# riveSunder/therldaisyworld

Hardware: AMD Instinct MI355X
Metric: cell-updates/sec (grid x batch), fused stencil+growth step (higher is better)
Workload: dtype f32

## Files before the change

### therldaisyworld_amd/csrc/dw_api.hip

```cpp
#include <hip/hip_runtime.h>

#include <cmath>
#include <cstdarg>
#include <cstdio>
#include <cstdlib>
#include <cstring>
#include <memory>
#include <new>
#include <type_traits>
#include <vector>

#include "../../include/daisyworld_hip.h"
#include "dw_kernels.hpp"
#include "dw_host_util.hpp"
#include "dw_plan.hpp"
#include "dw_series.hpp"

using namespace dw;

static thread_local char g_err[512] = "";

static int fail(int code, const char* fmt, ...) {
    va_list ap;
    va_start(ap, fmt);
// ... 439 lines not shown
        });
    } else {
        const int prec = p.precision == DW_PRECISION_F64 ? 2 : (ex ? 0 : 1);
        with_int<2, 0, 1>(prec, [&](auto PR) { generic(iL, iD, PR); });
    }
    HIPCHK(hipGetLastError());
    step_done(h, 0.0, true, true, constants);
    return DW_OK;
}

static int launch_forward_fused2_pw(dw_handle* h, const PairPw* row, StatsDev* trace) {
    const StepPlan& pl = h->plan;
    const StepOut o = step_out(h);
    const FusedGeom& g = pl.fgeom;
    const dim3 grid((unsigned)g.chunk * 8u);
    const plane_t *inL = h->L16[h->cur].get(), *inD = h->D16[h->cur].get();
    with_int<kFusedRot, kFusedOvl>(pl.fused_mode, [&](auto MODE) {
        hipLaunchKernelGGL((trace_pair_fast_pw<MODE>), grid, dim3(256), 0, h->stream, inL, inD, o.L, o.D, g, row, o.zero_me,
                           o.zero_n, trace);
    });
    HIPCHK(hipGetLastError());
    step_done(h, 0.0, false, true, true);
    return DW_OK;
}

static int temp_chunks(const dw_handle* h) {
    return (int)(((long long)h->prm.height * h->prm.width + kTempChunk - 1) / kTempChunk);
}
static size_t temp_part_bytes(const dw_handle* h) { return sizeof(TempPartial) * (size_t)h->prm.batch * temp_chunks(h); }

static int launch_temp_moments(dw_handle* h, bool current, double L, const PhysF64* row64, TempStatsDev* out) {
    const dw_params& p = h->prm;
    const int chunks = temp_chunks(h);
    const PhysF64 P = row64 ? PhysF64{} : make_f64(p, L);
    TempPartial* part = h->temp_part.get();
    auto reduce = [&](auto* iL, auto* iD) {
        with_bool(row64 != nullptr, [&](auto TABLE) {
            hipLaunchKernelGGL((temp_moments_pw<elem_t<decltype(iL)>, TABLE>), dim3((unsigned)chunks, (unsigned)p.batch), dim3(256),
                               0, h->stream, iL, iD, p.height, p.width, P, row64, part);
        });
    };
    if (current) with_planes(h, h->unq == OWN_CUR, h->cur, reduce);
    else with_derived_from(h, [&](auto* iL, auto* iD, auto) { reduce(iL, iD); });
    HIPCHK(hipGetLastError());
    hipLaunchKernelGGL(temp_moments_finish_pw, dim3((unsigned)((p.batch + 63) / 64)), dim3(64), 0, h->stream, part, p.batch, chunks,
                       (double)p.height * (double)p.width, out);
    HIPCHK(hipGetLastError());
    return DW_OK;
}

template <class F>
static auto with_fused_layout(const StepPlan& pl, F&& f) {
    if (pl.packed) return f(int_c<kFusedRot>{}, std::true_type{});
    return with_int<kFusedRot, kFusedRing, kFusedOvl>(pl.fused_mode, [&](auto MODE) { return f(MODE, std::false_type{}); });
}

static int launch_forward_fused2(dw_handle* h, double L1, double L2, unsigned int* pstats = nullptr,
                                 float thr_hi = 0.f, StatsDev* trace = nullptr) {
    const dw_params& p = h->prm;
    const StepPlan& pl = h->plan;
    const bool exact = p.precision == DW_PRECISION_EXACT;
    PhysF32 P1, P2;
    if (exact) derive_f32_pair(p, L1, L2, &P1, &P2);
    else { P1 = derive_f32(p, L1); P2 = derive_f32(p, L2); }
    const StepOut o = step_out(h);
    const FusedGeom& g = pl.fgeom;
    const dim3 grid((unsigned)g.chunk * 8u);
    const plane_t *inL = h->L16[h->cur].get(), *inD = h->D16[h->cur].get();
    auto exact_args = [&] {
        return FusedExactArgs{inL, inD, o.L, o.D, g, P1, lum_part(P2), o.zero_me, o.zero_n, pstats, thr_hi, make_f64(p, L1), L1, L2};
    };
    if (trace && exact) {
        const TraceExactArgs A{exact_args(), trace, h->sw.force_rescan ? 1 : 0};
        with_int<kFusedRot, kFusedOvl>(pl.fused_mode, [&](auto MODE) {
            with_bool(pl.sym_albedo, [&](auto SYM) {
                hipLaunchKernelGGL((trace_pair_exact<MODE, SYM>), grid, dim3(256), 0, h->stream, A);
            });
        });
    } else if (trace) {
        with_int<kFusedRot, kFusedOvl>(pl.fused_mode, [&](auto MODE) {
            hipLaunchKernelGGL((trace_pair_fast<MODE>), grid, dim3(256), 0, h->stream, inL, inD, o.L, o.D, g, P1, P2, o.zero_me,
                               o.zero_n, trace);
        });
    } else if (pl.fmt_planes && !pstats && !exact) {
        hipLaunchKernelGGL((step_stream_fused2_fmt_pw<kFusedOvl>), grid, dim3(256), 0, h->stream, inL, inD, o.L, o.D, g, P1, P2,
                           o.zero_me, o.zero_n);
    } else if (exact) {
        const FusedExactArgs A = exact_args();
        with_bool(pstats != nullptr, [&](auto STATS) {
            with_fused_layout(pl, [&](auto MODE, auto PACK) {
                with_bool(pl.sym_albedo, [&](auto SYM) {
                    hipLaunchKernelGGL((step_stream_fused2_exact<MODE, PACK, STATS, SYM>), grid, dim3(256), 0, h->stream, A);
                });
            });
        });
    } else {
        with_bool(pstats != nullptr, [&](auto STATS) {
            with_fused_layout(pl, [&](auto MODE, auto PACK) {
                hipLaunchKernelGGL((step_stream_fused2<MODE, PACK, STATS>), grid, dim3(256), 0, h->stream, inL, inD, o.L, o.D, g,
                                   P1, P2, o.zero_me, o.zero_n, pstats, thr_hi);
            });
        });
    }
    HIPCHK(hipGetLastError());
    step_done(h, L2, false);
    return DW_OK;
}

static int launch_agents(dw_handle* h, const int* d_action, int act_b, int act_n, bool standalone = false,
                         double* d_reward = nullptr, unsigned char* d_done = nullptr, unsigned char* d_ok = nullptr) {
    const dw_params& p = h->prm;
    if (p.n_agents == 0) return DW_OK;
    NEED(h->have_state, DW_ESTATE, "no state uploaded");
    NEED(h->have_agents, DW_ESTATE, "no agents uploaded (call dw_upload_agents or dw_init_random)");
    NEED(p.collision_mode == 0 || standalone, DW_EINVAL,
         "collision_mode=1: call dw_update_agents, apply the collision pass (it consumes the caller's RNG) to the "
         "downloaded agent states, upload them, then dw_step without actions");
    const int blocks = (p.batch + 63) / 64;
    with_planes(h, h->unq == OWN_CUR, h->cur, [&](auto* L, auto* D) {
        using T = elem_t<decltype(L)>;
        hipLaunchKernelGGL(agents_update<T>, dim3(blocks), dim3(64), 0, h->stream, L, D, h->idx.get(), h->st.get(), d_action,
                           act_b, act_n, p.batch, p.n_agents, p.height, p.width, p.agent_gamma,
                           p.collision_mode == 0 ? 1 : 0, d_reward, d_done, d_ok);
    });
    HIPCHK(hipGetLastError());
    return DW_OK;
}

static int stage_host_actions(dw_handle* h, const int32_t* action, int b, int n) {
    const dw_params& p = h->prm;
    NEED(b >= 0 && n >= 0 && b <= p.batch && n <= p.n_agents, DW_EINVAL,
         "action block %dx%d exceeds (B,N)=(%d,%d)", b, n, p.batch, p.n_agents);
    if ((size_t)b * n)
        HIPCHK(hipMemcpyAsync(h->action_tmp.get(), action, sizeof(int) * (size_t)b * n, hipMemcpyHostToDevice,
                              h->stream));
    return DW_OK;
}

static int clear_stats(dw_handle* h) {
    for (int i = 0; i < 2; ++i) HIPCHK(hipMemsetAsync(h->stats2[i].get(), 0, h->stats_bytes, h->stream));
    return DW_OK;
}

static void state_arrived(dw_handle* h, UnqOwner unq, UnqKind kind = UNQ_F64) {
    if (unq == OWN_CUR) h->unq_kind = kind;
    h->unq = unq;
    h->have_state = true;
    h->stepped = false;
    for (auto& sn : h->snap) sn.valid = false;
}

template <class T>
static auto init_random_into(dw_handle* h, uint64_t seed, T* L, T* D) {
    const dw_params& p = h->prm;
    if (int crc = clear_stats(h)) return crc;
    const int ncell = p.height * p.width;
    const dim3 g((unsigned)((ncell + kInitChunk - 1) / kInitChunk), (unsigned)p.batch);
    hipLaunchKernelGGL((init_random_cells<T>), g, dim3(256), 0, h->stream, L, D, ncell,
                       (long long)p.world_offset, (unsigned long long)seed, (float)p.light_proportion,
                       (float)p.dark_proportion, (float)p.initial_al, (float)p.initial_ad, h->stats2[h->sp].get());
    HIPCHK(hipGetLastError());
    if (p.n_agents) {
        const int bn = p.batch * p.n_agents;
        hipLaunchKernelGGL(init_random_agents, dim3((bn + 255) / 256), dim3(256), 0, h->stream, h->idx.get(), h->st.get(),
                           p.batch, p.n_agents, p.height, p.width, (long long)p.world_offset,
                           (unsigned long long)seed);
// ... 1613 lines not shown
        job(h->idx.get(), sn.idx.get(), sizeof(int) * 2 * bn);
        job(h->st.get(), sn.st.get(), sizeof(double) * bn);
    }
    if (sn.stepped && sn.unq != OWN_PREV) {
        job(h->L16[1 - h->cur].get(), sn.PL.get(), pb);
        job(h->D16[1 - h->cur].get(), sn.PD.get(), pb);
    }
    if (int rc = launch_copy_regions(h, J)) return rc;
    HIPCHK(hipMemsetAsync(h->stats2[1 - h->sp].get(), 0, h->stats_bytes, h->stream));
    h->unq = sn.unq;
    h->stepped = sn.stepped;
    h->L_last = sn.L_last;
    h->L_per_world = sn.L_per_world;
    h->P_per_world = sn.P_per_world;
    return DW_OK;
}

int dw_snapshot_save(dw_handle* h) { return dw_snapshot_save_slot(h, 0); }
int dw_snapshot_restore(dw_handle* h) { return dw_snapshot_restore_slot(h, 0); }


int dw_set_stream(dw_handle* h, void* hip_stream) {
    NEED(h, DW_EINVAL, "null handle");
    HIPCHK(hipSetDevice(h->prm.device));
    HIPCHK(hipStreamSynchronize(h->stream));
    if (h->own_stream) HIPCHK(hipStreamDestroy(h->stream));
    h->stream = reinterpret_cast<hipStream_t>(hip_stream);
    h->own_stream = false;
    return DW_OK;
}

int dw_sync(dw_handle* h) {
    NEED(h, DW_EINVAL, "null handle");
    HIPCHK(hipSetDevice(h->prm.device));
    HIPCHK(hipStreamSynchronize(h->stream));
    return DW_OK;
}

int dw_timer_start(dw_handle* h) {
    NEED(h, DW_EINVAL, "null handle");
    HIPCHK(hipSetDevice(h->prm.device));
    HIPCHK(hipEventRecord(h->ev0, h->stream));
    return DW_OK;
}

int dw_timer_stop(dw_handle* h, float* elapsed_ms) {
    NEED(h && elapsed_ms, DW_EINVAL, "null argument");
    HIPCHK(hipSetDevice(h->prm.device));
    HIPCHK(hipEventRecord(h->ev1, h->stream));
    HIPCHK(hipEventSynchronize(h->ev1));
    HIPCHK(hipEventElapsedTime(elapsed_ms, h->ev0, h->ev1));
    return DW_OK;
}

int dw_device_planes(dw_handle* h, int which, void** light, void** dark) {
    NEED(h && light && dark, DW_EINVAL, "null argument");
    NEED(which == DW_STATE_CURRENT || which == DW_STATE_PREVIOUS, DW_EINVAL, "bad state selector");
    const int buf = which == DW_STATE_CURRENT ? h->cur : 1 - h->cur;
    NEED(which != DW_STATE_CURRENT || cur_quantised(h), DW_ESTATE,
         "the current state is an un-quantised upload: it has no binary16 planes before the first step");
    *light = h->L16[buf].get();
    *dark = h->D16[buf].get();
    return DW_OK;
}

int dw_kernel_info(dw_handle* h, char* buf, size_t buflen) {
    NEED(h && buf && buflen, DW_EINVAL, "null argument");
    const dw_params& p = h->prm;
    const StepPlan& pl = h->plan;
    const char* prec = p.precision == DW_PRECISION_EXACT ? "exact" : (p.precision == DW_PRECISION_FAST ? "fast" : "f64");
    static const char* const halo_name[] = {"rotate", "dpp-old", "general", "packed"};
    if (pl.kind == STEP_STREAM) {
        const StripGeom& g = pl.sgeom;
        snprintf(buf, buflen,
                 "step_stream_%s<halo=%s> wave-strip=%dx256 cells, register window + DPP neighbours, %d-row blocks in "
                 "flight%s, %d strips, grid=%d x 256 threads (4 strips each), XCD-chunked",
                 prec, halo_name[pl.halo], g.SR,
                 p.precision == DW_PRECISION_EXACT ? DW_STREAM_RB_EXACT : DW_STREAM_RB_FAST,
                 p.precision == DW_PRECISION_EXACT ? ", in-wave float64 fix-up from an LDS queue" : "", g.nstrips,
                 g.chunk * 8);
        if (pl.allow_fuse) {
            const size_t n = std::strlen(buf);
            snprintf(buf + n, buflen - n, "; dw_step_n fuses step pairs (step_stream_fused2%s%s)",
                     p.precision == DW_PRECISION_EXACT ? "_exact" : "", pl.fmt_planes ? "_fmt_pw, format buffer accesses" : "");
        }
    } else if (pl.kind == STEP_TILED) {
        const int TR = (256 / pl.tcq) * pl.rpt;
        snprintf(buf, buflen,
                 "step_tiled<TCQ=%d,RPT=%d,%s> tile=%dx%d cells, %zu B LDS/workgroup, %d tiles, grid=%d x 256 threads, "
                 "XCD-chunked",
                 pl.tcq, pl.rpt, prec, TR, pl.tcq * 4, pl.tile_lds, pl.geom.ntiles, pl.geom.chunk * 8);
    } else {
        snprintf(buf, buflen, "step_generic<%s> one thread per cell, grid=(%d,%d) x 256 threads", prec,
                 (p.height * p.width + 255) / 256, p.batch);
    }
    {
        const size_t n = std::strlen(buf);
        snprintf(buf + n, buflen - n, pl.trace_pairs ? "; trace: step pairs" : "; trace: single steps");
    }
    {
        const size_t n = std::strlen(buf);
        snprintf(buf + n, buflen - n, pl.pw_stream ? "; per-world L: wave strips" : "; per-world L: generic");
    }
    {
        static const char* const form_name[] = {"launches per step", "workgroup (LDS)", "one wave per world"};
        const size_t n = std::strlen(buf);
        snprintf(buf + n, buflen - n, "; episode: %s; mlp episode: %s", form_name[episode_form(h)], form_name[episode_mlp_form(h)]);
    }
    {
        const size_t n = std::strlen(buf);
        snprintf(buf + n, buflen - n, "; ensemble episode: %s", ensemble_episode_wave(h) ? "one wave per world" : "launches per step");
    }
    {
        const size_t n = std::strlen(buf);
        snprintf(buf + n, buflen - n, "; episode trace: %s", episode_trace_wave(h) ? "one wave per world" : "launches per step");
    }
    if (pl.first_stream) {
        const size_t n = std::strlen(buf);
        snprintf(buf + n, buflen - n, "; first step: wave-strip=%dx256", pl.first_geom.SR);
    }
    if (h->sw.text[0]) {
        const size_t n = std::strlen(buf);
        snprintf(buf + n, buflen - n, "; switches[%s]", h->sw.text);
    }
    {
        const size_t n = std::strlen(buf);
        snprintf(buf + n, buflen - n, "; per-world constants: %s",
                 ensemble_pairs(h) ? "step pairs" : (pl.pw_stream ? "wave strips" : "generic"));
    }
    return DW_OK;
}

int dw_audit_tie_bound(dw_handle* h, double L, double out[4]) {
    NEED(h && out, DW_EINVAL, "null argument");
    const dw_params& p = h->prm;
    HIPCHK(hipSetDevice(p.device));
    NEED(h->have_state && cur_quantised(h), DW_ESTATE, "the audit needs a quantised current state");
    const StepPlan& pl = h->plan;
    int rc = ensure_scratch(h, 4 * sizeof(unsigned long long));
    if (rc) return rc;
    unsigned long long* d = reinterpret_cast<unsigned long long*>(h->scratch.get());
    HIPCHK(hipMemsetAsync(d, 0, 4 * sizeof(unsigned long long), h->stream));
    const dim3 g((unsigned)((p.height * p.width + 255) / 256), (unsigned)p.batch);
    hipLaunchKernelGGL(tie_audit, g, dim3(256), 0, h->stream, h->L16[h->cur].get(), h->D16[h->cur].get(), p.height, p.width,
                       derive_f32(p, L), make_f64(p, L), d, pl.sym_albedo && pl.kind == STEP_STREAM ? 1 : 0);
    HIPCHK(hipGetLastError());
    unsigned long long r[4];
    HIPCHK(hipMemcpyAsync(r, d, sizeof(r), hipMemcpyDeviceToHost, h->stream));
    HIPCHK(hipStreamSynchronize(h->stream));
    std::memcpy(&out[0], &r[0], sizeof(double));
    std::memcpy(&out[1], &r[1], sizeof(double));
    out[2] = (double)r[2];
    out[3] = (double)r[3];
    return DW_OK;
}

int dw_last_fixup_count(dw_handle* h, uint64_t* count) {
    NEED(h && count, DW_EINVAL, "null argument");
    HIPCHK(hipSetDevice(h->prm.device));
    std::vector<StatsDev> st((size_t)h->prm.batch + 1);
    HIPCHK(hipMemcpyAsync(st.data(), h->stats2[h->sp].get(), sizeof(StatsDev) * st.size(), hipMemcpyDeviceToHost, h->stream));
    HIPCHK(hipStreamSynchronize(h->stream));
    unsigned long long v = st[h->prm.batch].sum_l;
    for (int b = 0; b < h->prm.batch; ++b) v += st[b].reserved;
    *count = v;
    return DW_OK;
}
// ... 3 lines not shown
```

### therldaisyworld_amd/csrc/dw_kernels.hpp

```cpp
#pragma once
#include "dw_common.hpp"
#include "dw_step_generic.hpp"
#include "dw_step_tiled.hpp"
#include "dw_step_stream.hpp"
#include "dw_step_fused.hpp"
#include "dw_step_first.hpp"
#include "dw_step_per_world.hpp"
#include "dw_step_fused_pw.hpp"
#include "dw_episode.hpp"
#include "dw_episode_wave.hpp"
#include "dw_agents.hpp"
#include "dw_state_io.hpp"
#include "dw_agents_fused.hpp"
#include "dw_temp_moments.hpp"
#include "dw_episode_wave_pw.hpp"
#include "dw_episode_wave_stats_pw.hpp"
```

### therldaisyworld_amd/csrc/dw_plan.hpp

```cpp
#pragma once
#include <climits>
#include <cmath>
#include <cstddef>
#include <cstdio>
#include <cstdlib>
#include <cstring>

#include "../../include/daisyworld_hip.h"
#include "dw_types.hpp"

namespace dw {

struct Switches {
    bool no_sym = false, no_pack = false, no_fuse = false, no_ring = false, no_fmt_planes = false, no_episode_kernel = false,
         no_episode_wave = false, no_agent_fuse = false, no_agent_preapply = false, first_f64 = false,
         first_generic = false, force_rescan = false, test_hooks = false;
    int pack_min_strips = -1, strip_rows = 0, tile_rpt = 0, queue_cap = -1, mismatch_cap = -1, trace_rows = 0;
    double first_slack = -1.0;
    char kernel[16] = {0};
    char text[256] = {0};
};
inline const char* test_hook(const char* name) {
    return std::getenv("DW_TEST_HOOKS") ? std::getenv(name) : nullptr;
}
inline Switches read_switches() {
    Switches w;
    auto note = [&](const char* name, const char* val) {
        const size_t n = std::strlen(w.text);
        snprintf(w.text + n, sizeof(w.text) - n, "%s%s%s%s", n ? " " : "", name, val ? "=" : "", val ? val : "");
    };
    auto flag = [&](const char* name, bool& dst) { if (std::getenv(name)) { dst = true; note(name, nullptr); } };
    auto num = [&](const char* name, int& dst, bool test) {
        if (const char* e = test ? test_hook(name) : std::getenv(name)) { dst = std::atoi(e); note(name, e); }
    };
    w.test_hooks = std::getenv("DW_TEST_HOOKS") != nullptr;
    flag("DW_NO_SYM", w.no_sym); flag("DW_NO_PACK", w.no_pack); flag("DW_NO_FUSE", w.no_fuse); flag("DW_NO_RING", w.no_ring);
    flag("DW_NO_FMT_PLANES", w.no_fmt_planes);
    flag("DW_NO_EPISODE_KERNEL", w.no_episode_kernel); flag("DW_NO_EPISODE_WAVE", w.no_episode_wave);
    flag("DW_NO_AGENT_FUSE", w.no_agent_fuse); flag("DW_NO_AGENT_PREAPPLY", w.no_agent_preapply);
    flag("DW_FIRST_STEP_F64", w.first_f64); flag("DW_FIRST_GENERIC", w.first_generic);
    num("DW_PACK_MIN_STRIPS", w.pack_min_strips, false); num("DW_STRIP_ROWS", w.strip_rows, false);
    num("DW_TILE_RPT", w.tile_rpt, false);
    num("DW_TEST_QUEUE_CAP", w.queue_cap, true); num("DW_TEST_MISMATCH_CAP", w.mismatch_cap, true);
    num("DW_TEST_TRACE_ROWS", w.trace_rows, true);
    if (test_hook("DW_TEST_FORCE_RESCAN")) { w.force_rescan = true; note("DW_TEST_FORCE_RESCAN", nullptr); }
    if (const char* e = test_hook("DW_TEST_FIRST_SLACK")) { w.first_slack = std::atof(e); note("DW_TEST_FIRST_SLACK", e); }
    if (const char* e = std::getenv("DW_KERNEL")) { snprintf(w.kernel, sizeof(w.kernel), "%s", e); note("DW_KERNEL", e); }
    return w;
}

inline dw_params with_world_params(dw_params p, const dw_world_params& w) {
    p.p = w.p; p.g = w.g; p.S = w.S; p.sigma = w.sigma; p.gamma = w.gamma; p.q = w.q; p.q2 = w.q2; p.dt = w.dt;
    p.albedo_bare = w.albedo_bare; p.albedo_light = w.albedo_light; p.albedo_dark = w.albedo_dark;
    p.temp_optimal = w.temp_optimal;
    return p;
}
inline dw_world_params world_params_of(const dw_params& p) {
    return dw_world_params{p.p, p.g, p.S, p.sigma, p.gamma, p.q, p.q2, p.dt, p.albedo_bare, p.albedo_light, p.albedo_dark,
                           p.temp_optimal};
}
inline bool albedo_symmetric(double bare, double light, double dark) { return (dark - bare) == -(light - bare); }
inline bool worlds_symmetric(const dw_world_params* worlds, size_t B) {
    for (size_t b = 0; b < B; ++b)
        if (!albedo_symmetric(worlds[b].albedo_bare, worlds[b].albedo_light, worlds[b].albedo_dark)) return false;
    return true;
}

inline PhysF64 make_f64(const dw_params& p, double L) {
    PhysF64 P;
    P.p = p.p; P.g = p.g; P.S = p.S; P.sigma = p.sigma; P.gamma = p.gamma; P.q = p.q; P.q2 = p.q2;
    P.dt = p.dt; P.ab = p.albedo_bare; P.al = p.albedo_light; P.ad = p.albedo_dark;
    P.To = p.temp_optimal; P.L = L;
    const double e1 = std::exp(-1.0), e2 = std::exp(-2.0);
    const double s = 1.0 + 4.0 * e1 + 4.0 * e2;
    P.w0 = 1.0 / s; P.w1 = e1 / s; P.w2 = e2 / s;
    return P;
}

inline double cbeta_host(const dw_params& p) {
    const double cbeta = p.g * p.temp_optimal * p.temp_optimal;
    return cbeta > 1e-30 ? 1.0 / std::sqrt(cbeta) : 0x1p60;
}

inline void split_hi_lo(double v, double scale, float* hi, float* lo) {
    const double h = std::nearbyint(v * scale) / scale;
    *hi = (float)h;
    *lo = (float)(v - h);
}

inline float round_up(double v) {
    const float f = (float)v;
    return (double)f < v ? std::nextafterf(f, INFINITY) : f;
}

struct EConst { double c0l, c0d; };
inline EConst e_const(const dw_params& p, double L) {
    const double To4 = std::pow(p.temp_optimal, 4), K = p.S * L / p.sigma;
    const double e0 = K * (1.0 - p.albedo_bare * p.p) / To4 - 1.0;
    return EConst{e0 + p.q2 * (p.albedo_bare * p.p - p.albedo_light) / To4,
                  e0 + p.q2 * (p.albedo_bare * p.p - p.albedo_dark) / To4};
}

struct TieChain {
    double emin, emax, vlo;
    bool admissible;
    double ew;
    double kbmax;
    double pu, safety;
};
inline TieChain tie_chain(const dw_params& p, const EConst& c, double a1, double a2, double a3, double a4, double de) {
    const double u = std::ldexp(1.0, -24), kmax = 1000.0;
    TieChain t;
    const double pos = (std::fmax(a1, 0.0) + std::fmax(a2, 0.0)) * 8 * kmax + (std::fmax(a3, 0.0) + std::fmax(a4, 0.0)) * kmax;
    const double neg = (std::fmin(a1, 0.0) + std::fmin(a2, 0.0)) * 8 * kmax + (std::fmin(a3, 0.0) + std::fmin(a4, 0.0)) * kmax;
    t.emax = std::fmax(c.c0l, c.c0d) + pos;
    t.emin = std::fmin(c.c0l, c.c0d) + neg;
    const double vmin = 1.0 + t.emin, vmax = 1.0 + t.emax;
    t.admissible = vmin > 0.02;
    t.vlo = std::fmax(vmin, 0.02);
    const double smax = std::sqrt(std::fmax(vmax, t.vlo));
// ... 39 lines not shown
    P.a1 = (float)((double)P.a1h + P.a1l); P.a2 = (float)((double)P.a2h + P.a2l);
    P.a3 = (float)((double)P.a3h + P.a3l); P.a4 = (float)((double)P.a4h + P.a4l);
    P.c0ls = (float)((double)P.c0lh + P.c0ll); P.c0ds = (float)((double)P.c0dh + c0dl);
    const double kbe = cbeta_host(p);
    P.kbeta = (float)kbe;
    const PhysF64 P64 = make_f64(p, L);
    P.dw0 = (float)(p.dt * P64.w0); P.dw1 = (float)(p.dt * P64.w1); P.dw2 = (float)(p.dt * P64.w2);
    P.p = (float)p.p; P.ck = p.dt != 0.0 ? (float)(0.001 / p.dt) : 0.f;
    P.ngamma = (float)(-p.gamma);
    const double u = std::ldexp(1.0, -24);
    const double lo_mag = std::ldexp(1.0, -(hb + 1)) * 18.0 * kmax + std::ldexp(1.0, -(hb + 1));
    const double de_abs = 6.0 * u * lo_mag + 1e-9;
    const TieChain t = tie_chain(p, c0, a1, a2, a3, a4, de_abs);
    auto e_over_D2 = [&](double e) {
        const double v = std::fmax(1.0 + e, t.vlo), sv = std::sqrt(v), yv = std::sqrt(sv);
        const double D = kbe * (yv + 1.0) * (sv + 1.0);
        return std::fabs(e) / (D * D);
    };
    const double Ae = 2.0 * de_abs * std::fmax(e_over_D2(t.emin), e_over_D2(t.emax));
    double A0 = t.safety * (kmax * std::fabs(p.dt) * t.kbmax * Ae + 2e-6);
    if (!t.admissible) A0 = 1.0;
    const double eA = t.safety * 13.0 * u;
    const double eK0d = t.safety * (6.0 * std::fabs(p.p) + t.pu + t.kbmax + 8.0 * std::fabs(p.gamma)) * u;
    const double eK1d = t.safety * ((6.0 * std::fabs(p.p) + t.pu) * u + t.kbmax * (u + 2.0 * t.ew));
    P.tie_lo = (float)(0.5 - A0);
    if ((double)P.tie_lo > 0.5 - A0) P.tie_lo = std::nextafterf(P.tie_lo, -INFINITY);
    P.eA = round_up(eA);
    const float eK0 = round_up(eK0d), eK1 = round_up(eK1d);
    P.eK0s = p.dt < 0.0 ? eK0 : -eK0;
    P.eK1s = p.dt < 0.0 ? eK1 : -eK1;
    P.neK1s = -P.eK1s;
    P.eK01s = (float)((double)P.eK0s + (double)P.eK1s);
    if (std::fabs((double)P.eK01s) < std::fabs((double)P.eK0s + (double)P.eK1s))
        P.eK01s = std::nextafterf(P.eK01s, P.eK01s < 0.f ? -1.f : 1.f);
    return P;
}

inline void derive_f32_pair(const dw_params& p, double L1, double L2, PhysF32* P1, PhysF32* P2) {
    const PhysF32 a = derive_f32(p, L1), b = derive_f32(p, L2);
    const int hb = a.hi_bits < b.hi_bits ? a.hi_bits : b.hi_bits;
    *P1 = derive_f32(p, L1, hb);
    *P2 = derive_f32(p, L2, hb);
    const float tie_lo = P1->tie_lo < P2->tie_lo ? P1->tie_lo : P2->tie_lo;
    P1->tie_lo = tie_lo;
    P2->tie_lo = tie_lo;
}

inline FirstStepBound derive_first_bound(const dw_params& p, double L, const PhysF32& P, bool from_f64,
                                         double test_slack = -1.0) {
    const double u = std::ldexp(1.0, -24), iota = from_f64 ? u : 0.0;
    const double kmax = 1000.0;
    const double a1 = std::fabs((double)P.a1), a2 = std::fabs((double)P.a2), a3 = std::fabs((double)P.a3), a4 = std::fabs((double)P.a4);
    const EConst c0 = e_const(p, L);
    const double c0m = std::fmax(std::fabs(c0.c0l), std::fabs(c0.c0d));
    const double Mmax = (a1 + a2) * 8 * kmax + (a3 + a4) * kmax;
    const double de_max = (8.0 * u + iota) * Mmax + u * c0m;
    const TieChain t = tie_chain(p, c0, P.a1, P.a2, P.a3, P.a4, de_max);
    const double kbe = cbeta_host(p);
    const double Dmin = kbe * (std::sqrt(std::sqrt(t.vlo)) + 1.0) * (std::sqrt(t.vlo) + 1.0);
    const double kK = 5.0 * u + iota;
    const double safety = t.safety, pu = t.pu, kbmax = t.kbmax;
    FirstStepBound B;
    B.a1 = round_up(a1); B.a2 = round_up(a2); B.a3 = round_up(a3); B.a4 = round_up(a4);
    B.c_de = round_up(safety * (8.0 * u + iota) * (1.0 + 8.0 * u));
    B.c_c0 = round_up(safety * u * c0m);
    B.eK0 = round_up(safety * (pu + (kK + 2.0 * u) * std::fabs(p.p) + kbmax * u + ((kK + 3.0 * u) + u) * std::fabs(p.gamma)));
    B.eK1 = round_up(safety * (pu + (kK + 2.0 * u) * std::fabs(p.p) + kbmax * (u + 2.0 * t.ew)));
    B.cW = round_up(safety * 2.0 * kbmax / Dmin);
    B.eA = round_up(safety * ((kK + 3.0 * u) + u + (kK + u)));
    B.cS = round_up(safety * u);
    B.slack = t.admissible ? 4e-6f : 1.0f;
    if (test_slack > (double)B.slack) B.slack = (float)test_slack;
    return B;
}

enum StepKind { STEP_GENERIC, STEP_TILED, STEP_STREAM };
struct StepPlan {
    StepKind kind = STEP_GENERIC;
    int halo = 0;
    bool packed = false;
    bool allow_fuse = false;
    int fused_mode = kFusedOvl;
    bool fmt_planes = false;
    bool trace_pairs = false;
    bool sym_albedo = false;
    int tcq = 0, rpt = 0;
    Geom geom{};
    size_t tile_lds = 0;
    StripGeom sgeom{};
    FusedGeom fgeom{};
    int first_prec = 2;
    bool first_stream = false;
    FirstGeom first_geom{};
    bool need_fixq = false;
    bool pw_stream = false;
};

inline int halo_form(int W) { return W < 256 ? 3 : (W == 256 ? 0 : (W % 256 == 0 ? 1 : 2)); }

inline int strip_rows(long groups, int H, long target) {
    int sr = 64;
    while (sr > 8 && groups * ((H + sr - 1) / sr) < target) sr >>= 1;
    return H < sr ? H : sr;
}

inline int strip_rows_or_override(const Switches& sw, int cap, long groups, int H, long target) {
    if (sw.strip_rows < 1) return strip_rows(groups, H, target);
    const int want = sw.strip_rows < cap ? sw.strip_rows : cap;
    return H < want ? H : want;
}

inline StepPlan plan_steps(const dw_params& p, const Switches& sw) {
    StepPlan s;
    s.sym_albedo = albedo_symmetric(p.albedo_bare, p.albedo_light, p.albedo_dark) && !sw.no_sym;
    s.halo = halo_form(p.width);
    const int lpw = p.width / 4, wpr = lpw ? 64 / lpw : 0;
    const bool pack_shape = p.width >= 8 && p.width < 256 && wpr >= 1 && wpr * lpw * 10 >= 64 * 7 && !sw.no_pack;
    const long pack_strips = pack_shape ? (long)((p.batch + wpr - 1) / wpr) * ((p.height + 63) / 64) : 0;
    const bool packable = pack_shape && pack_strips >= (sw.pack_min_strips >= 0 ? sw.pack_min_strips : 512);
    const bool quads = p.precision != DW_PRECISION_F64 && p.width % 4 == 0;
    if (quads && (p.width >= 256 || packable) && std::strcmp(sw.kernel, "tiled") != 0) {
        s.kind = STEP_STREAM;
        s.packed = p.width < 256;
        StripGeom& g = s.sgeom;
        g.B = p.batch; g.H = p.height; g.W = p.width;
        g.ncs = (p.width + 255) / 256;
        g.lpw = s.packed ? lpw : 64;
        g.wpr = s.packed ? wpr : 1;
        const long groups = s.packed ? (p.batch + wpr - 1) / wpr : p.batch;
        g.SR = strip_rows_or_override(sw, INT_MAX, groups * g.ncs, p.height, 2048);
        g.nrs = (p.height + g.SR - 1) / g.SR;
        g.nstrips = (int)(groups * g.nrs * g.ncs);
        g.nwg = (g.nstrips + 3) / 4;
        g.chunk = (g.nwg + 7) / 8;
        g.qcap = kWaveQueueCap;
        int mcap = kMismatchCap;
        if (sw.queue_cap >= 0 && sw.queue_cap < kWaveQueueCap) g.qcap = sw.queue_cap;
        if (sw.mismatch_cap >= 0 && sw.mismatch_cap < kMismatchCap) mcap = sw.mismatch_cap;
        g.force_rescan = sw.force_rescan ? 1 : 0;
        s.allow_fuse = !sw.no_fuse;
        const bool ring = p.width == 1024 && !sw.no_ring;
        s.fused_mode = p.width <= 256 ? kFusedRot : (ring ? kFusedRing : kFusedOvl);
        FusedGeom& f = s.fgeom;
        f.B = p.batch; f.H = p.height; f.W = p.width;
        f.SR = g.SR;
        f.nrs = g.nrs;
        f.lpw = g.lpw; f.wpr = g.wpr;
        f.cols_per_strip = p.width <= 256 ? 256 : (ring ? 1024 : 248);
        f.ncs = s.packed ? 1 : (p.width + f.cols_per_strip - 1) / f.cols_per_strip;
        f.nstrips = (int)(groups * f.nrs * f.ncs);
        f.nwg = ring ? f.nstrips : (f.nstrips + 3) / 4;
        f.chunk = (f.nwg + 7) / 8;
        f.qcap = g.qcap;
        f.mcap = mcap;
        f.sure_need = 9 * p.n_agents + 9 * mcap + 1;
        s.trace_pairs = s.allow_fuse && !s.packed && s.fused_mode != kFusedRing;
        s.fmt_planes = p.precision == DW_PRECISION_FAST && s.allow_fuse && !s.packed && s.fused_mode == kFusedOvl && !sw.no_fmt_planes &&
                       (size_t)p.height * p.width * sizeof(plane_t) < ((size_t)1 << 31);
    } else if (quads && p.width >= 64) {
        s.kind = STEP_TILED;
        const int Wq = p.width / 4;
        if (Wq >= 64) {
            s.tcq = 64; s.rpt = 4;
            if (sw.tile_rpt == 2 || sw.tile_rpt == 4 || sw.tile_rpt == 8) s.rpt = sw.tile_rpt;
        }
        else if (Wq >= 32) { s.tcq = 32; s.rpt = 4; }
        else { s.tcq = 16; s.rpt = 2; }
        const int TR = (256 / s.tcq) * s.rpt;
        Geom& g = s.geom;
        g.B = p.batch; g.H = p.height; g.W = p.width; g.Wq = Wq;
        g.tiles_r = (p.height + TR - 1) / TR;
        g.tiles_c = (Wq + s.tcq - 1) / s.tcq;
        g.ntiles = p.batch * g.tiles_r * g.tiles_c;
        g.chunk = (g.ntiles + 7) / 8;
        g.qcap = kMaxFix;
        if (sw.queue_cap >= 0 && sw.queue_cap < kMaxFix) g.qcap = sw.queue_cap;
        s.tile_lds = (size_t)2 * (TR + 2) * (s.tcq + 2) * 4 * sizeof(float);
    }
    s.need_fixq = p.precision == DW_PRECISION_EXACT && s.kind == STEP_TILED;
    s.pw_stream = s.kind == STEP_STREAM && !s.packed;
    s.first_prec = p.precision == DW_PRECISION_FAST ? 1 : (p.precision == DW_PRECISION_EXACT && !sw.first_f64 ? 3 : 2);
    s.first_stream = (p.width % 256 == 0 || s.kind == STEP_STREAM) && s.first_prec != 2 && !sw.first_generic;
    if (s.first_stream) {
        FirstGeom& fg = s.first_geom;
        fg.B = p.batch; fg.H = p.height; fg.W = p.width;
        fg.lpw = s.packed ? lpw : 64;
        fg.wpr = s.packed ? wpr : 1;
        fg.ncs = s.packed ? 1 : (p.width + 255) / 256;
        const long groups = s.packed ? (p.batch + fg.wpr - 1) / fg.wpr : p.batch;
        fg.SR = strip_rows_or_override(sw, 64, groups * fg.ncs, p.height, 4096);
        fg.nrs = (p.height + fg.SR - 1) / fg.SR;
        fg.nstrips = (int)(groups * fg.nrs * fg.ncs);
    }
    return s;
}

}
```

### therldaisyworld_amd/csrc/dw_types.hpp

```cpp
#pragma once

namespace dw {

typedef _Float16 plane_t;

struct PhysF64 {
    double p, g, S, sigma, gamma, q, q2, dt;
    double ab, al, ad, To;
    double L;
    double w0, w1, w2;
};

typedef float dw_f32x2 __attribute__((ext_vector_type(2)));
#define DW_PAIR(lo_name, hi_name, pair_name) \
    union { struct { float lo_name, hi_name; }; dw_f32x2 pair_name; }

struct PhysF32 {
    DW_PAIR(a1h, a2h, a12h);
    DW_PAIR(a3h, a4h, a34h);
    DW_PAIR(a1l, a2l, a12l);
    DW_PAIR(a3l, a4l, a34l);
    DW_PAIR(c0lh, c0ll, c0l);
    DW_PAIR(c0dh, dc0l, c0d);
    DW_PAIR(a1, a2, a12);
    DW_PAIR(a3, a4, a34);
    DW_PAIR(c0ls, c0ds, c0s);
    DW_PAIR(dw0, dw1, dw01);
    DW_PAIR(dw2, kbeta, dw2kb);
    DW_PAIR(p, ck, pck);
    DW_PAIR(eK1s, eK0s, eKs);
    DW_PAIR(ngamma, tie_lo, gt);
    DW_PAIR(neK1s, eK01s, eKb);
    float eA;
    int hi_bits;
};
static_assert(sizeof(PhysF32) == 32 * sizeof(float), "PhysF32 layout");

struct PhysLumF32 {
    dw_f32x2 a12h, a12l, c0l, c0d, a12, c0s;
};

struct FirstStepBound {
    float a1, a2, a3, a4;
    float c_de, c_c0;
    float eK0, eK1, cW, eA, cS, slack;
};

struct PairPw {
    PhysF32 P1, P2;
};
static_assert(sizeof(PairPw) == 2 * sizeof(PhysF32), "PairPw layout");

struct StatsDev {
    unsigned int max_k;
    unsigned int reserved;
    unsigned long long sum_l;
    unsigned long long sum_d;
};

struct Geom {
    int B, H, W;
    int Wq;
    int tiles_r, tiles_c;
    int ntiles;
    int chunk;
    int qcap;
};

struct StripGeom {
    int B, H, W;
    int SR;
    int ncs, nrs;
    int nstrips;
    int nwg;
    int chunk;
    int qcap;
    int lpw, wpr;
    int force_rescan;
};

struct FusedGeom {
    int B, H, W;
    int SR;
    int ncs, nrs;
    int nstrips, nwg, chunk;
    int cols_per_strip;
    int qcap, mcap;
    int lpw, wpr;
    int sure_need;
};

struct FirstGeom {
    int B, H, W;
    int SR;
    int ncs, nrs;
    int nstrips;
    int lpw, wpr;
};

enum { kFusedOvl = 0, kFusedRot = 1, kFusedRing = 2 };
constexpr int kWaveQueueCap = 256;
constexpr int kMismatchCap = 64;
constexpr int kMaxFix = 1024;
constexpr int kNumQueues = 256;

}
```

Baseline: 800.7 billion.

## Add fused step-pair kernel using full 256-column strips with LDS halo table

Adds a new fused two-step kernel for fast precision that uses full 256-column strips with no overlap. The column halo for the intermediate step is precomputed into a per-wave LDS table, which removes the redundant halo columns the overlapping 248-column strips recompute. The kernel is selected by default when the width is a multiple of 256 (but not 1024) and the strip height is small enough. In exchange it adds a serial halo pre-pass per strip and more LDS traffic and wave-level syncs.

Result: slower. 775.8 billion (-3.1%).

```diff
diff --git a/therldaisyworld_amd/csrc/dw_api.hip b/therldaisyworld_amd/csrc/dw_api.hip
--- a/therldaisyworld_amd/csrc/dw_api.hip
+++ b/therldaisyworld_amd/csrc/dw_api.hip
@@ -545,6 +545,10 @@
             hipLaunchKernelGGL((trace_pair_fast<MODE>), grid, dim3(256), 0, h->stream, inL, inD, o.L, o.D, g, P1, P2, o.zero_me,
                                o.zero_n, trace);
         });
+    } else if (pl.full_strips && !pstats && !exact) {
+        const FullGeom& u = pl.full_geom;
+        hipLaunchKernelGGL(step_stream_fused2_full_fmt_pw, dim3((unsigned)u.chunk * 8u), dim3(256), 0, h->stream, inL, inD, o.L, o.D,
+                           u, P1, P2, o.zero_me, o.zero_n);
     } else if (pl.fmt_planes && !pstats && !exact) {
         hipLaunchKernelGGL((step_stream_fused2_fmt_pw<kFusedOvl>), grid, dim3(256), 0, h->stream, inL, inD, o.L, o.D, g, P1, P2,
                            o.zero_me, o.zero_n);
@@ -2324,7 +2328,8 @@
         if (pl.allow_fuse) {
             const size_t n = std::strlen(buf);
             snprintf(buf + n, buflen - n, "; dw_step_n fuses step pairs (step_stream_fused2%s%s)",
-                     p.precision == DW_PRECISION_EXACT ? "_exact" : "", pl.fmt_planes ? "_fmt_pw, format buffer accesses" : "");
+                     p.precision == DW_PRECISION_EXACT ? "_exact" : "", pl.full_strips ? "_full_fmt_pw, full 256-column strips, format buffer accesses"
+                                    : (pl.fmt_planes ? "_fmt_pw, format buffer accesses" : ""));
         }
     } else if (pl.kind == STEP_TILED) {
         const int TR = (256 / pl.tcq) * pl.rpt;
diff --git a/therldaisyworld_amd/csrc/dw_kernels.hpp b/therldaisyworld_amd/csrc/dw_kernels.hpp
--- a/therldaisyworld_amd/csrc/dw_kernels.hpp
+++ b/therldaisyworld_amd/csrc/dw_kernels.hpp
@@ -4,6 +4,7 @@
 #include "dw_step_tiled.hpp"
 #include "dw_step_stream.hpp"
 #include "dw_step_fused.hpp"
+#include "dw_step_fused_full.hpp"
 #include "dw_step_first.hpp"
 #include "dw_step_per_world.hpp"
 #include "dw_step_fused_pw.hpp"
diff --git a/therldaisyworld_amd/csrc/dw_plan.hpp b/therldaisyworld_amd/csrc/dw_plan.hpp
--- a/therldaisyworld_amd/csrc/dw_plan.hpp
+++ b/therldaisyworld_amd/csrc/dw_plan.hpp
@@ -12,7 +12,8 @@
 namespace dw {
 
 struct Switches {
-    bool no_sym = false, no_pack = false, no_fuse = false, no_ring = false, no_fmt_planes = false, no_episode_kernel = false,
+    bool no_sym = false, no_pack = false, no_fuse = false, no_ring = false, no_fmt_planes = false, no_full_strips = false,
+         no_episode_kernel = false,
          no_episode_wave = false, no_agent_fuse = false, no_agent_preapply = false, first_f64 = false,
          first_generic = false, force_rescan = false, test_hooks = false;
     int pack_min_strips = -1, strip_rows = 0, tile_rpt = 0, queue_cap = -1, mismatch_cap = -1, trace_rows = 0;
@@ -35,7 +36,7 @@
     };
     w.test_hooks = std::getenv("DW_TEST_HOOKS") != nullptr;
     flag("DW_NO_SYM", w.no_sym); flag("DW_NO_PACK", w.no_pack); flag("DW_NO_FUSE", w.no_fuse); flag("DW_NO_RING", w.no_ring);
-    flag("DW_NO_FMT_PLANES", w.no_fmt_planes);
+    flag("DW_NO_FMT_PLANES", w.no_fmt_planes); flag("DW_NO_FULL_STRIPS", w.no_full_strips);
     flag("DW_NO_EPISODE_KERNEL", w.no_episode_kernel); flag("DW_NO_EPISODE_WAVE", w.no_episode_wave);
     flag("DW_NO_AGENT_FUSE", w.no_agent_fuse); flag("DW_NO_AGENT_PREAPPLY", w.no_agent_preapply);
     flag("DW_FIRST_STEP_F64", w.first_f64); flag("DW_FIRST_GENERIC", w.first_generic);
@@ -241,6 +242,8 @@
     bool allow_fuse = false;
     int fused_mode = kFusedOvl;
     bool fmt_planes = false;
+    bool full_strips = false;
+    FullGeom full_geom{};
     bool trace_pairs = false;
     bool sym_albedo = false;
     int tcq = 0, rpt = 0;
@@ -316,6 +319,17 @@
         s.trace_pairs = s.allow_fuse && !s.packed && s.fused_mode != kFusedRing;
         s.fmt_planes = p.precision == DW_PRECISION_FAST && s.allow_fuse && !s.packed && s.fused_mode == kFusedOvl && !sw.no_fmt_planes &&
                        (size_t)p.height * p.width * sizeof(plane_t) < ((size_t)1 << 31);
+        s.full_strips = s.fmt_planes && p.width % 256 == 0 && p.width != 1024 && !sw.no_full_strips && f.SR <= kFullMaxSR;
+        if (s.full_strips) {
+            FullGeom& u = s.full_geom;
+            u.B = p.batch; u.H = p.height; u.W = p.width;
+            u.SR = f.SR;
+            u.nrs = f.nrs;
+            u.ncs = p.width / 256;
+            u.nstrips = (int)((long)p.batch * u.nrs * u.ncs);
+            u.nwg = (u.nstrips + 3) / 4;
+            u.chunk = (u.nwg + 7) / 8;
+        }
     } else if (quads && p.width >= 64) {
         s.kind = STEP_TILED;
         const int Wq = p.width / 4;
diff --git a/therldaisyworld_amd/csrc/dw_step_fused_full.hpp b/therldaisyworld_amd/csrc/dw_step_fused_full.hpp
--- /dev/null
+++ b/therldaisyworld_amd/csrc/dw_step_fused_full.hpp
@@ -0,0 +1,199 @@
+#pragma once
+#include "dw_step_fused.hpp"
+
+namespace dw {
+
+constexpr int kFullTableRows = kFullMaxSR + 5;
+constexpr int kFullSlots = 66;
+constexpr int kFullField = kFullTableRows + kFullSlots;
+constexpr int kFullWaveFloats = 8 * kFullField;
+
+typedef __attribute__((address_space(3))) volatile float full_lds_word;
+
+__device__ __forceinline__ void full_lds_sync() {
+    __builtin_amdgcn_fence(__ATOMIC_RELEASE, "wavefront");
+    __builtin_amdgcn_wave_barrier();
+    __builtin_amdgcn_fence(__ATOMIC_ACQUIRE, "wavefront");
+}
+
+__device__ __forceinline__ void full_halo_cells(const PhysF32& P, dw_f32x2 li, dw_f32x2 di, dw_f32x2 El, dw_f32x2 Cl,
+                                                dw_f32x2 Ed, dw_f32x2 Cd, dw_f32x2& vl, dw_f32x2& vd) {
+#pragma clang fp contract(off)
+    const GrowthT<dw_f32x2> g = growth_t<kFastSplit, dw_f32x2, false>(P, li, di, El, Cl, Ed, Cd);
+    vl = finish_fast_t<dw_f32x2>(li, g.dKl, g.fl);
+    vd = finish_fast_t<dw_f32x2>(di, g.dKd, g.fd);
+}
+
+__global__ __launch_bounds__(256) __attribute__((amdgpu_waves_per_eu(DW_FUSED_FAST_WAVES, DW_FUSED_FAST_WAVES)))
+void step_stream_fused2_full_fmt_pw(const plane_t* __restrict__ inL, const plane_t* __restrict__ inD,
+                                    plane_t* __restrict__ outL, plane_t* __restrict__ outD, FullGeom G, PhysF32 P1, PhysF32 P2,
+                                    unsigned long long* __restrict__ zero_me, int zero_n) {
+#pragma clang fp contract(off)
+    __shared__ __attribute__((aligned(16))) float s_full[4 * kFullWaveFloats];
+    const int bid = blockIdx.x;
+    const int wg = (bid & 7) * G.chunk + (bid >> 3);
+    if (wg >= G.nwg) return;
+    const int tid = threadIdx.x, wv = tid >> 6, lane = tid & 63;
+    if (wg == 0)
+        for (int i = tid; i < zero_n; i += 256) zero_me[i] = 0ull;
+    const int s = __builtin_amdgcn_readfirstlane(wg * 4 + wv);
+    if (s >= G.nstrips) return;
+    const int spw = G.nrs * G.ncs;
+    const int b = s / spw;
+    const int sw = s - b * spw;
+    const int rs = sw / G.ncs, cs = sw - rs * G.ncs;
+    const int r0 = rs * G.SR;
+    const int nr = min(G.SR, G.H - r0);
+    const int c0 = cs * 256;
+
+    const unsigned int world_bytes = (unsigned int)(G.H * G.W) * 2u;
+    const dw_i32x4 fmt_inL = fmt_plane_rsrc(inL, b, world_bytes), fmt_inD = fmt_plane_rsrc(inD, b, world_bytes);
+    const dw_i32x4 fmt_outL = fmt_plane_rsrc(outL, b, world_bytes), fmt_outD = fmt_plane_rsrc(outD, b, world_bytes);
+    const int fmt_col = (c0 + 4 * lane) * 2, fmt_row = G.W * 2;
+
+    float* const tbl = s_full + wv * kFullWaveFloats;
+    constexpr int F = kFullField;
+
+    {
+        const int gA = ((c0 == 0 ? G.W : c0) - 4) * 2, gB = c0 * 2, gC = (c0 + 252) * 2, gD = (c0 + 256 == G.W ? 0 : c0 + 256) * 2;
+        for (int base = 0; base < nr + 4; base += 64) {
+            const int t = base + lane;
+            if (t < nr + 4) {
+                const int ro = wrap_near2(r0 - 2 + t, G.H) * fmt_row;
+                const float4 aL = fmt_load4(fmt_inL, ro + gA, 0), bL = fmt_load4(fmt_inL, ro + gB, 0);
+                const float4 cL = fmt_load4(fmt_inL, ro + gC, 0), dL = fmt_load4(fmt_inL, ro + gD, 0);
+                const float4 aD = fmt_load4(fmt_inD, ro + gA, 0), bD = fmt_load4(fmt_inD, ro + gB, 0);
+                const float4 cD = fmt_load4(fmt_inD, ro + gC, 0), dD = fmt_load4(fmt_inD, ro + gD, 0);
+                float* const T = tbl + t;
+                T[2 * F] = aL.w; T[3 * F] = aD.w; T[6 * F] = dL.x; T[7 * F] = dD.x;
+                T[0 * F] = aL.z + bL.x; T[1 * F] = aD.z + bD.x; T[4 * F] = cL.w + dL.y; T[5 * F] = cD.w + dD.y;
+            }
+        }
+    }
+    for (int base = ((nr + 1) >> 6) << 6; base >= 0; base -= 64) {
+        const int t = 1 + base + lane;
+        const bool mine = t <= nr + 2;
+        dw_f32x2 vl = dw_f32x2(0.f), vd = dw_f32x2(0.f);
+        full_lds_sync();
+        if (mine) {
+            auto pr = [&](int f, int r) { return dw_f32x2{tbl[f * F + r], tbl[(f + 4) * F + r]}; };
+            const dw_f32x2 El = pr(0, t) + (pr(2, t - 1) + pr(2, t + 1)), Cl = pr(0, t - 1) + pr(0, t + 1);
+            const dw_f32x2 Ed = pr(1, t) + (pr(3, t - 1) + pr(3, t + 1)), Cd = pr(1, t - 1) + pr(1, t + 1);
+            full_halo_cells(P1, pr(2, t), pr(3, t), El, Cl, Ed, Cd, vl, vd);
+        }
+        full_lds_sync();
+        if (mine) {
+            float* const T = tbl + t + 2;
+            T[0 * F] = vl.x; T[1 * F] = vd.x; T[4 * F] = vl.y; T[5 * F] = vd.y;
+        }
+    }
+    full_lds_sync();
+
+    full_lds_word* const t0 = (full_lds_word*)tbl;
+    full_lds_word* const w0 = t0 + kFullTableRows + lane;
+    auto table_row_to_slot = [&](auto HALF, int row) {
+        constexpr int h = decltype(HALF)::value;
+        const full_lds_word* const tr = t0 + row;
+        const float a = tr[(h + 0) * F], b = tr[(h + 1) * F], c = tr[(h + 4) * F], d = tr[(h + 5) * F];
+        full_lds_sync();
+        w0[1 + (h + 0) * F] = a; w0[1 + (h + 1) * F] = b; w0[1 + (h + 4) * F] = c; w0[1 + (h + 5) * F] = d;
+    };
+    auto exchange = [&](auto HALF, int next_row, float lx, float lw, float dx, float dw, float& ll, float& dl, float& lr,
+                        float& dr) {
+        constexpr int h = decltype(HALF)::value;
+        full_lds_sync();
+        w0[2 + (h + 0) * F] = lw; w0[2 + (h + 1) * F] = dw;
+        w0[(h + 4) * F] = lx; w0[(h + 5) * F] = dx;
+        full_lds_sync();
+        ll = w0[1 + (h + 0) * F]; dl = w0[1 + (h + 1) * F];
+        lr = w0[1 + (h + 4) * F]; dr = w0[1 + (h + 5) * F];
+        table_row_to_slot(HALF, next_row);
+    };
+    using H0 = std::integral_constant<int, 0>;
+    using H2 = std::integral_constant<int, 2>;
+    table_row_to_slot(H2{}, 0);
+    table_row_to_slot(H0{}, 3);
+    struct RawIn { float4 l, d; };
+    auto load_raw = [&](int rr) -> RawIn {
+        rr = min(rr, r0 + nr + 1);
+        rr = rr < 0 ? rr + G.H : rr;
+        rr = rr >= G.H ? rr - G.H : rr;
+        RawIn w;
+        w.l = fmt_load4(fmt_inL, fmt_col, rr * fmt_row);
+        w.d = fmt_load4(fmt_inD, fmt_col, rr * fmt_row);
+        return w;
+    };
+    auto pin_edge_sums = [&](Row4& L, Row4& D) {
+        asm volatile("" : "+v"(L.h2[0]), "+v"(L.h2[3]), "+v"(D.h2[0]), "+v"(D.h2[3]));
+    };
+    Row4 IL[3], ID[3], SL[3], SD[3];
+    {
+        const RawIn p0 = load_raw(r0 - 2), p1 = load_raw(r0 - 1), p2 = load_raw(r0);
+        auto first_rows = [&](const RawIn& p, int row, Row4& L, Row4& D) {
+            const float4 l = widen4(p.l), d = widen4(p.d);
+            float ll, dl, lr, dr;
+            exchange(H2{}, row + 1, l.x, l.w, d.x, d.w, ll, dl, lr, dr);
+            L = make_row(l, ll, lr);
+            D = make_row(d, dl, dr);
+        };
+        first_rows(p0, 0, IL[0], ID[0]);
+        first_rows(p1, 1, IL[1], ID[1]);
+        first_rows(p2, 2, IL[2], ID[2]);
+    }
+    using U0 = std::integral_constant<int, 0>;
+    using U1 = std::integral_constant<int, 1>;
+    using U2 = std::integral_constant<int, 2>;
+    auto iter = [&](auto U, auto D1, auto D2, int j) {
+        constexpr int u = decltype(U)::value;
+        constexpr bool do1 = decltype(D1)::value, do2 = decltype(D2)::value;
+        RawIn nx;
+        if (do1) nx = load_raw(r0 + j);
+        if constexpr (!do1) {
+            Row4 &ml = SL[(u + 1) % 3], &md = SD[(u + 1) % 3];
+            asm volatile("" : "+v"(ml.x[0]), "+v"(ml.x[1]), "+v"(ml.x[2]), "+v"(ml.x[3]), "+v"(md.x[0]), "+v"(md.x[1]), "+v"(md.x[2]), "+v"(md.x[3]));
+        }
+        __builtin_amdgcn_sched_barrier(0);
+        float l1[4], d1[4], l2[4], d2[4];
+        if (do2)
+            cells4<false, false, bool>(P2, SL[u], SL[(u + 1) % 3], SL[(u + 2) % 3], SD[u], SD[(u + 1) % 3], SD[(u + 2) % 3], l2, d2,
+                                       nullptr);
+        if (do1)
+            cells4<false, false, bool>(P1, IL[(u + 2) % 3], IL[u], IL[(u + 1) % 3], ID[(u + 2) % 3], ID[u], ID[(u + 1) % 3], l1, d1,
+                                       nullptr);
+        if (do2) {
+            fmt_store4(fmt_outL, fmt_col, (r0 + j - 4) * fmt_row, make_float4(l2[0], l2[1], l2[2], l2[3]));
+            fmt_store4(fmt_outD, fmt_col, (r0 + j - 4) * fmt_row, make_float4(d2[0], d2[1], d2[2], d2[3]));
+        }
+        if (do1) {
+            float ll, dl, lr, dr;
+            exchange(H0{}, j + 3, l1[0], l1[3], d1[0], d1[3], ll, dl, lr, dr);
+            SL[u] = make_row(make_float4(l1[0], l1[1], l1[2], l1[3]), ll, lr);
+            SD[u] = make_row(make_float4(d1[0], d1[1], d1[2], d1[3]), dl, dr);
+            __builtin_amdgcn_sched_barrier(0);
+            const float4 il = widen4(nx.l), id = widen4(nx.d);
+            exchange(H2{}, j + 3, il.x, il.w, id.x, id.w, ll, dl, lr, dr);
+            IL[(u + 2) % 3] = make_row(il, ll, lr);
+            ID[(u + 2) % 3] = make_row(id, dl, dr);
+            pin_edge_sums(IL[(u + 2) % 3], ID[(u + 2) % 3]);
+        }
+    };
+    using Yes = std::true_type;
+    using No = std::false_type;
+    iter(U1{}, Yes{}, No{}, 1);
+    iter(U2{}, Yes{}, No{}, 2);
+    iter(U0{}, Yes{}, No{}, 3);
+    const int jend = nr + 2;
+    int j = 4;
+    for (; j + 2 <= jend; j += 3) {
+        iter(U1{}, Yes{}, Yes{}, j);
+        iter(U2{}, Yes{}, Yes{}, j + 1);
+        iter(U0{}, Yes{}, Yes{}, j + 2);
+    }
+    if (j <= jend) { iter(U1{}, Yes{}, Yes{}, j); ++j; }
+    if (j <= jend) { iter(U2{}, Yes{}, Yes{}, j); ++j; }
+    if (j % 3 == 1) iter(U1{}, No{}, Yes{}, j);
+    else if (j % 3 == 2) iter(U2{}, No{}, Yes{}, j);
+    else iter(U0{}, No{}, Yes{}, j);
+}
+
+}
diff --git a/therldaisyworld_amd/csrc/dw_types.hpp b/therldaisyworld_amd/csrc/dw_types.hpp
--- a/therldaisyworld_amd/csrc/dw_types.hpp
+++ b/therldaisyworld_amd/csrc/dw_types.hpp
@@ -90,6 +90,13 @@
     int sure_need;
 };
 
+struct FullGeom {
+    int B, H, W;
+    int SR;
+    int ncs, nrs;
+    int nstrips, nwg, chunk;
+};
+
 struct FirstGeom {
     int B, H, W;
     int SR;
@@ -101,6 +108,7 @@
 enum { kFusedOvl = 0, kFusedRot = 1, kFusedRing = 2 };
 constexpr int kWaveQueueCap = 256;
 constexpr int kMismatchCap = 64;
+constexpr int kFullMaxSR = 123;
 constexpr int kMaxFix = 1024;
 constexpr int kNumQueues = 256;
 
```
